# bede/kindel

Hardware: NVIDIA H100
Metric: aligned bases/sec through pileup+consensus (higher is better)
Workload: dtype int32

## Files before the change

include/kindel_b200.h:

```cpp
#ifndef KINDEL_B200_H
#define KINDEL_B200_H

#include <stdint.h>

#ifdef __cplusplus
extern "C" {
#endif

#define KDL_ABI_VERSION 2
#define KDL_NCOL 19
#define KDL_NVOTE_COL 7
#define KDL_COMPLEX 0x80000000u
#define KDL_HARD 0x40000000u
#define KDL_LEN_MASK 0x0000ffffu
#define KDL_NM_SHIFT 16
#define KDL_NM_MASK 0x7fu
#define KDL_TILE 512
#define KDL_FAST_MAXLEN 8192
#define KDL_TILE_MAXOPS 64
#define KDL_TILE_MAXREACH 1024

enum kdl_col {
    KDL_W_A = 0, KDL_W_C, KDL_W_G, KDL_W_T, KDL_W_N,
    KDL_DEL = 5, KDL_INS = 6, KDL_CLIP_STARTS = 7, KDL_CLIP_ENDS = 8,
// ... 39 lines not shown
    const uint32_t* off;
    const uint32_t* qpos;
} kdl_qmask;

typedef struct kdl_diag {
    int32_t status;
    int32_t reserved;
    int64_t read;
    int32_t nibble;
    int32_t op_index;
} kdl_diag;

int kdl_abi_version(void);
const char* kdl_status_string(int status);
int64_t kdl_launch_count(void);

int kdl_pileup(const kdl_batch* batch, int32_t* counts, int64_t n_slots, int32_t* ins_events,
               int32_t* err_flag, void* stream);

#define KDL_PILEUP_FRESH_WEIGHTS 1
#define KDL_PILEUP_ZERO_REST 2
int kdl_pileup_range(const kdl_batch* batch, int32_t* counts, int64_t n_slots, int64_t slot_lo,
                     int64_t slot_hi, int32_t flags, int32_t* ins_events, int32_t* err_flag, void* stream);

int kdl_unmask(const kdl_batch* batch, const kdl_qmask* qmask, int32_t* counts, int64_t n_slots, void* stream);

int kdl_diagnose(const kdl_batch* batch, kdl_diag* diag_dev, void* stream);

int kdl_vote(const int32_t* counts, int64_t n_slots, int64_t min_depth_ceil, uint8_t* calls,
             void* stream);

int kdl_vote_iupac(const int32_t* counts, int64_t n_slots, int64_t min_depth_ceil, double threshold, uint8_t* calls,
                   void* stream);

int kdl_derive(const int32_t* counts, int64_t n_slots, int32_t* out, void* stream);

int kdl_cdr_flags(const int32_t* counts, int64_t n_slots, int64_t slot_lo, int64_t slot_hi,
                  double clip_decay_threshold, uint8_t* flags, uint8_t* bases, void* stream);

int64_t kdl_assemble_scratch_words(int64_t n_slots);
int kdl_assemble(const uint8_t* calls, int64_t n_slots, const int64_t* contig_slot, const int32_t* contig_len,
                 int32_t n_contigs, const int64_t* ins_slot, const uint32_t* ins_off, const uint8_t* ins_bytes,
                 int64_t n_ins, uint32_t* block_sums, uint32_t* offsets, uint8_t* out, void* stream);

int kdl_consensus_qual(const int32_t* counts, const uint8_t* calls, int64_t n_slots, uint8_t* qual, void* stream);

// ... 76 lines not shown
```

kindel_b200/_ffi.py:

```python
from __future__ import annotations

import ctypes as C
import os

from . import build as _build

c_i32p = C.POINTER(C.c_int32)
c_u32p = C.POINTER(C.c_uint32)
c_i64p = C.POINTER(C.c_int64)
c_u8p = C.POINTER(C.c_uint8)

KDL_NCOL = 19
KDL_NVOTE_COL = 7
KDL_COMPLEX = 0x80000000
KDL_HARD = 0x40000000
KDL_LEN_MASK = 0xFFFF
KDL_NM_SHIFT = 16
KDL_NM_MASK = 0x7F
KDL_TILE_MAXOPS = 64
KDL_TILE_MAXREACH = 1024
KDL_TILE = 512
KDL_PILEUP_FRESH_WEIGHTS = 1
KDL_PILEUP_ZERO_REST = 2
KDL_FAST_MAXLEN = 8192
# ... 50 lines not shown
        ("slice_lo", C.c_int64 * 16),
        ("slice_hi", C.c_int64 * 16),
        ("counter", C.c_void_p),
    ]


class KdlDiag(C.Structure):
    _fields_ = [
        ("status", C.c_int32),
        ("reserved", C.c_int32),
        ("read", C.c_int64),
        ("nibble", C.c_int32),
        ("op_index", C.c_int32),
    ]


_PROTOTYPES = {
    "kdl_abi_version": (C.c_int, []),
    "kdl_status_string": (C.c_char_p, [C.c_int]),
    "kdl_launch_count": (C.c_int64, []),
    "kdl_pileup": (C.c_int, [C.POINTER(KdlBatch), C.c_void_p, C.c_int64, C.c_void_p, C.c_void_p, C.c_void_p]),
    "kdl_pileup_range": (C.c_int, [C.POINTER(KdlBatch), C.c_void_p, C.c_int64, C.c_int64, C.c_int64, C.c_int32,
                                   C.c_void_p, C.c_void_p, C.c_void_p]),
    "kdl_diagnose": (C.c_int, [C.POINTER(KdlBatch), C.c_void_p, C.c_void_p]),
    "kdl_unmask": (C.c_int, [C.POINTER(KdlBatch), C.POINTER(KdlQmask), C.c_void_p, C.c_int64, C.c_void_p]),
    "kdl_vote": (C.c_int, [C.c_void_p, C.c_int64, C.c_int64, C.c_void_p, C.c_void_p]),
    "kdl_vote_iupac": (C.c_int, [C.c_void_p, C.c_int64, C.c_int64, C.c_double, C.c_void_p, C.c_void_p]),
    "kdl_derive": (C.c_int, [C.c_void_p, C.c_int64, C.c_void_p, C.c_void_p]),
    "kdl_cdr_flags": (C.c_int, [C.c_void_p, C.c_int64, C.c_int64, C.c_int64, C.c_double, C.c_void_p, C.c_void_p, C.c_void_p]),
    "kdl_assemble_scratch_words": (C.c_int64, [C.c_int64]),
    "kdl_assemble": (C.c_int, [C.c_void_p, C.c_int64, C.c_void_p, C.c_void_p, C.c_int32, C.c_void_p, C.c_void_p,
                               C.c_void_p, C.c_int64, C.c_void_p, C.c_void_p, C.c_void_p, C.c_void_p]),
    "kdl_consensus_qual": (C.c_int, [C.c_void_p, C.c_void_p, C.c_int64, C.c_void_p, C.c_void_p]),
    "kdl_assemble_qual": (C.c_int, [C.c_void_p, C.c_void_p, C.c_int64, C.c_void_p, C.c_void_p, C.c_int64, C.c_void_p,
                                    C.c_void_p]),
    "kdl_variant_scratch_words": (C.c_int64, [C.c_int64]),
    "kdl_variant_count": (C.c_int, [C.c_void_p, C.c_int64, C.c_void_p, C.c_void_p, C.c_int32, C.c_int64, C.c_double,
                                    C.c_void_p, C.c_void_p]),
    "kdl_variant_scatter": (C.c_int, [C.c_void_p, C.c_int64, C.c_void_p, C.c_void_p, C.c_int32, C.c_int64, C.c_double,
                                      C.c_void_p, C.c_int64, C.c_void_p, C.c_void_p, C.c_void_p, C.c_void_p]),
    "kdl_vote_peers": (C.c_int, [C.POINTER(C.c_void_p), C.c_int32, C.c_int64, C.c_int64, C.c_int64, C.c_int64,
                                 C.c_void_p, C.c_void_p, C.c_void_p]),
    "kdl_vote_peers_sparse": (C.c_int, [C.POINTER(C.c_void_p), C.POINTER(C.c_int64), C.POINTER(C.c_int64), C.c_int32,
                                        C.c_int64, C.c_int64, C.c_int64, C.c_int64, C.c_void_p, C.c_void_p, C.c_void_p]),
    "kdl_exchange_signal": (C.c_int, [C.POINTER(KdlExchange), C.c_int32, C.c_void_p]),
    "kdl_exchange_vote": (C.c_int, [C.POINTER(KdlExchange), C.c_int64, C.c_int64, C.c_int32, C.c_void_p]),
# ... 64 lines not shown
```

kindel_b200/csrc/api.cu:

```cuda
#include <atomic>
#include <cstdio>
#include <cstdlib>
#include <cstring>
#include <new>

#include "kdl_common.cuh"
#include "pileup_general.cu"
#include "pileup_simple.cu"
#include "pileup_tile.cu"
#include "pileup_mask.cu"
#include "vote.cu"
#include "assemble.cu"
#include "variants.cu"

namespace {

std::atomic<long long> g_launches{0};

inline int grid_for(long long items, int per_block, int cap) {
    long long g = (items + per_block - 1) / per_block;
    if (g < 1) g = 1;
    if (g > cap) g = cap;
    return (int)g;
}
// ... 11 lines not shown
    const int dev = current_device();
    int n = cache[dev].load(std::memory_order_relaxed);
    if (n <= 0) {
        if (cudaDeviceGetAttribute(&n, cudaDevAttrMultiProcessorCount, dev) != cudaSuccess || n <= 0) n = 132;
        cache[dev].store(n, std::memory_order_relaxed);
    }
    return n;
}

template <int kFlush, bool kCx>
inline int ensure_tile_smem() {
    static std::atomic<int> done[kMaxDevices];
    const int dev = current_device();
    if (done[dev].load(std::memory_order_acquire)) return KDL_OK;
    if (cudaFuncSetAttribute(kdl::pileup_tile_kernel<kFlush, kCx>, cudaFuncAttributeMaxDynamicSharedMemorySize,
                             (int)sizeof(kdl::TileSmem<kdl::TileCfg<kCx>>)) != cudaSuccess)
        return KDL_ERR_CUDA;
    done[dev].store(1, std::memory_order_release);
    return KDL_OK;
}

template <int kFlush, bool kCx>
inline int launch_tile(const kdl_batch& b, int32_t* counts, long long n_slots, long long tile_lo, long long n_tiles,
                       int split, int zero_rest, cudaStream_t st) {
    int rc = ensure_tile_smem<kFlush, kCx>();
    if (rc != KDL_OK) return rc;
    const long long units = n_tiles * split, max_grid = (long long)sm_count() * 2;
    const long long grid = units < max_grid ? units : max_grid;
    kdl::pileup_tile_kernel<kFlush, kCx><<<(unsigned)grid, kdl::W_THREADS, sizeof(kdl::TileSmem<kdl::TileCfg<kCx>>), st>>>(
        b, counts, n_slots, b.tile_index, tile_lo, n_tiles, split, zero_rest);
    return KDL_OK;
}

inline int check_launch() {
    g_launches.fetch_add(1, std::memory_order_relaxed);
    return cudaGetLastError() == cudaSuccess ? KDL_OK : KDL_ERR_CUDA;
}

int validate_batch(const kdl_batch* b) {
    if (!b || b->n_reads < 0 || b->n_contigs < 0 || b->n_hard < 0 || b->n_complex < b->n_hard)
        return KDL_ERR_INVALID_ARG;
    if (b->n_reads > 0 && (!b->ref_start || !b->seq_off || !b->l_seq || !b->seq4 ||
                           !b->contig_read_off || !b->contig_len || !b->contig_slot))
        return KDL_ERR_INVALID_ARG;
    if ((b->n_hard > 0 && !b->hard_idx) || (b->n_complex > 0 && !b->complex_idx)) return KDL_ERR_INVALID_ARG;
    if (b->reach_right < b->max_simple_len || b->reach_left < 0) return KDL_ERR_INVALID_ARG;
    return KDL_OK;
}

}

extern "C" {

int kdl_abi_version(void) { return KDL_ABI_VERSION; }

const char* kdl_status_string(int status) {
    switch (status) {
        case KDL_OK: return "ok";
        case KDL_ERR_INVALID_ARG: return "invalid argument";
        case KDL_ERR_CUDA: return "CUDA error";
        case KDL_ERR_NO_DEVICE: return "no CUDA device";
        case KDL_ERR_INDEX: return "IndexError: read walks off the contig or off its SEQ";
        case KDL_ERR_KEY: return "KeyError: base outside A,C,G,T,N in an M or S op";
        default: return "unknown status";
    }
}

int64_t kdl_launch_count(void) { return g_launches.load(std::memory_order_relaxed); }

int kdl_pileup(const kdl_batch* batch, int32_t* counts, int64_t n_slots, int32_t* ins_events,
               int32_t* err_flag, void* stream) {
    return kdl_pileup_range(batch, counts, n_slots, 0, n_slots, 0, ins_events, err_flag, stream);
}

int kdl_pileup_range(const kdl_batch* batch, int32_t* counts, int64_t n_slots, int64_t slot_lo,
                     int64_t slot_hi, int32_t flags, int32_t* ins_events, int32_t* err_flag, void* stream) {
    int rc = validate_batch(batch);
    if (rc != KDL_OK) return rc;
    if (!counts || !err_flag || n_slots <= 0 || slot_lo < 0 || slot_hi > n_slots || slot_lo > slot_hi)
        return KDL_ERR_INVALID_ARG;
    const bool tileable = (n_slots % KDL_TILE) == 0 && (slot_lo % KDL_TILE) == 0 && (slot_hi % KDL_TILE) == 0;
    if ((slot_lo & 3) || (slot_hi & 3)) return KDL_ERR_INVALID_ARG;
    cudaStream_t st = (cudaStream_t)stream;
    const int cap = sm_count() * 8;
    const bool has_tile_reads = batch->n_reads > batch->n_hard;
    const bool tiled = has_tile_reads && tileable && batch->reads_sorted && batch->tile_index &&
                       batch->reach_right > 0 && batch->reach_right <= KDL_FAST_MAXLEN + KDL_TILE_MAXREACH;
    const bool fresh = (flags & KDL_PILEUP_FRESH_WEIGHTS) != 0;
    const long long tile_lo = slot_lo / KDL_TILE, n_tiles = (slot_hi - slot_lo) / KDL_TILE;
    int split = 1;
    if (tiled && n_tiles > 0) {
        const long long slots = (long long)sm_count() * 2;
        if (n_tiles < slots) {
            long long want = (slots + n_tiles - 1) / n_tiles;
            const long long deep = batch->n_reads / (n_tiles * 256);
            if (want > deep) want = deep;
            split = (int)(want < 1 ? 1 : (want > 32 ? 32 : want));
        }
        if (const char* ev = getenv("KDL_SPLIT")) { const int v = atoi(ev); if (v >= 1 && v <= 64) split = v; }
    }
    bool cx_by_atomics = (batch->n_complex - batch->n_hard) * 16 < batch->n_reads;
    if (const char* ev = getenv("KDL_CX")) cx_by_atomics = !strcmp(ev, "atomics") ? true : (!strcmp(ev, "pieces") ? false : cx_by_atomics);
    const int zero_in_k1 = (tiled && split == 1 && fresh && n_tiles > 0 && (flags & KDL_PILEUP_ZERO_REST)) ? 1 : 0;
    const int zero_from = (fresh && !(tiled && split == 1)) ? 0 : 5;
    const int zero_to = ((flags & KDL_PILEUP_ZERO_REST) && !zero_in_k1) ? KDL_NCOL : 5;
    if (zero_to > zero_from && slot_hi > slot_lo) {
        kdl::zero_cols_kernel<<<sm_count() * 4, 256, 0, st>>>(counts, n_slots, zero_from, zero_to, slot_lo, slot_hi);
        if ((rc = check_launch()) != KDL_OK) return rc;
    }
    if (batch->n_reads == 0) return KDL_OK;
    if (tiled) {
        if (n_tiles > 0) {
            kdl::tile_index_kernel<<<(unsigned)((n_tiles * 32 + 255) / 256), 256, 0, st>>>(*batch, tile_lo, n_tiles,
                                                                                          batch->tile_index);
            if ((rc = check_launch()) != KDL_OK) return rc;
            const bool cx = batch->n_complex > batch->n_hard && !cx_by_atomics;
            if (split > 1) {
                rc = cx ? launch_tile<kdl::F_ATOMIC, true>(*batch, counts, n_slots, tile_lo, n_tiles, split, 0, st)
                        : launch_tile<kdl::F_ATOMIC, false>(*batch, counts, n_slots, tile_lo, n_tiles, split, 0, st);
            } else if (fresh) {
                rc = cx ? launch_tile<kdl::F_STORE, true>(*batch, counts, n_slots, tile_lo, n_tiles, 1, zero_in_k1, st)
                        : launch_tile<kdl::F_STORE, false>(*batch, counts, n_slots, tile_lo, n_tiles, 1, zero_in_k1, st);
            } else {
                rc = cx ? launch_tile<kdl::F_ADD, true>(*batch, counts, n_slots, tile_lo, n_tiles, 1, 0, st)
                        : launch_tile<kdl::F_ADD, false>(*batch, counts, n_slots, tile_lo, n_tiles, 1, 0, st);
            }
            if (rc != KDL_OK) return rc;
            if ((rc = check_launch()) != KDL_OK) return rc;
        }
        if (batch->n_complex > batch->n_hard) {
            if (cx_by_atomics)
                kdl::pileup_events_kernel<8><<<(unsigned)((batch->n_complex + 31) / 32), 256, 0, st>>>(
                    *batch, counts, n_slots, ins_events, 1);
            else
                kdl::pileup_events_kernel<1><<<(unsigned)((batch->n_complex + 255) / 256), 256, 0, st>>>(
                    *batch, counts, n_slots, ins_events, 0);
            if ((rc = check_launch()) != KDL_OK) return rc;
        }
        if (batch->n_hard > 0) {
            const int grid = grid_for(batch->n_hard, 8, cap);
            kdl::pileup_general_kernel<<<grid, 256, 0, st>>>(*batch, batch->hard_idx, batch->n_hard, counts, n_slots,
                                                            ins_events, err_flag);
            if ((rc = check_launch()) != KDL_OK) return rc;
        }
    } else {
        if (batch->n_reads > batch->n_complex) {
            const int grid = grid_for(batch->n_reads, 8, cap);
            kdl::pileup_simple_atomic_kernel<<<grid, 256, 0, st>>>(*batch, counts, n_slots, err_flag);
            if ((rc = check_launch()) != KDL_OK) return rc;
        }
        if (batch->n_complex > 0) {
            const int grid = grid_for(batch->n_reads, 8, cap);
            kdl::pileup_general_kernel<<<grid, 256, 0, st>>>(*batch, nullptr, batch->n_reads, counts, n_slots,
                                                            ins_events, err_flag);
            if ((rc = check_launch()) != KDL_OK) return rc;
        }
    }
    return KDL_OK;
}

int kdl_unmask(const kdl_batch* batch, const kdl_qmask* qmask, int32_t* counts, int64_t n_slots, void* stream) {
    int rc = validate_batch(batch);
    if (rc != KDL_OK) return rc;
    if (!qmask || !counts || n_slots <= 0 || qmask->n_reads < 0 || qmask->n_bases < 0 || qmask->n_reads > batch->n_reads)
        return KDL_ERR_INVALID_ARG;
    if (qmask->n_reads == 0) return KDL_OK;
    if (!qmask->read_idx || !qmask->off || !qmask->qpos) return KDL_ERR_INVALID_ARG;
    const long long grid = (qmask->n_reads + kdl::kQThreads - 1) / kdl::kQThreads;
    kdl::unmask_kernel<<<(unsigned)grid, kdl::kQThreads, 0, (cudaStream_t)stream>>>(*batch, *qmask, counts, n_slots);
    return check_launch();
}

int kdl_diagnose(const kdl_batch* batch, kdl_diag* diag_dev, void* stream) {
    int rc = validate_batch(batch);
    if (rc != KDL_OK) return rc;
    if (!diag_dev) return KDL_ERR_INVALID_ARG;
    cudaStream_t st = (cudaStream_t)stream;
// ... 268 lines not shown
```

kindel_b200/csrc/kdl_common.cuh:

```cuda
#pragma once
#include <cuda_runtime.h>
#include <stdint.h>

#include "../../include/kindel_b200.h"

#ifndef KDL_HOST_EMU
#define KDL_DYNAMIC_SMEM(name) extern __shared__ __align__(16) unsigned char name[]
#else
#define KDL_DYNAMIC_SMEM(name) extern unsigned char name[]
#endif

namespace kdl {

__device__ __forceinline__ int nib2col(int nib) {
    const unsigned long long lut = 0x4FFFFFF3FFF2F10FULL;
    int v = (int)((lut >> (nib * 4)) & 0xF);
    return v == 0xF ? -1 : v;
}

__device__ __forceinline__ int nibble_at(const uint32_t* __restrict__ seq, long long q) {
    return (int)((seq[q >> 3] >> (28 - 4 * (int)(q & 7))) & 0xFu);
}

__device__ __forceinline__ long long complex_len(uint32_t lraw) {
    return (lraw & KDL_HARD) ? (long long)(lraw & 0x3fffffffu) : (long long)(lraw & KDL_LEN_MASK);
}

__device__ __forceinline__ long long pyindex(long long i, long long n) {
    if (i < 0) i += n;
    return (i < 0 || i >= n) ? -1 : i;
}

__device__ __forceinline__ int find_contig(const int64_t* __restrict__ off, int n_contigs, long long r) {
    int lo = 0, hi = n_contigs;
    while (lo < hi) {
        int mid = (lo + hi) >> 1;
        if (off[mid + 1] > r) hi = mid; else lo = mid + 1;
    }
    return lo;
}

__device__ __forceinline__ int base_vote(int a, int c, int g, int t, int n, int* freq, int* raw_base) {
    int best = a, code = 0;
    if (t > best) { best = t; code = 3; }
    if (g > best) { best = g; code = 2; }
    if (c > best) { best = c; code = 1; }
    if (n > best) { best = n; code = 4; }
    const int ties = (a == best) + (c == best) + (g == best) + (t == best) + (n == best);
    if (best == 0) code = 4;
    *freq = best;
    *raw_base = code;
    return (best != 0 && ties > 1) ? 4 : code;
}

__device__ __forceinline__ unsigned vote_slot(int a, int c, int g, int t, int n, int del, int ins,
                                              long long depth_next, long long min_depth_ceil) {
    const long long depth = (long long)a + c + g + t;
    if (2ll * del > depth) return (1u << 4) | 4u;
    if (depth < min_depth_ceil) return (2u << 4) | 4u;
    const long long thr = depth < depth_next ? depth : depth_next;
    const unsigned change = (2ll * ins > thr) ? 3u : 0u;
    int freq, raw;
// ... 53 lines not shown
```

kindel_b200/csrc/pileup_general.cu:

```cuda
#include "kdl_common.cuh"

namespace kdl {

__global__ void __launch_bounds__(256)
pileup_general_kernel(kdl_batch b, const uint32_t* __restrict__ list, long long n_list, int32_t* __restrict__ counts,
                      long long n_slots, int32_t* __restrict__ ins_events, int32_t* __restrict__ err_flag) {
    const int lane = threadIdx.x & 31;
    const long long warp0 = ((long long)blockIdx.x * blockDim.x + threadIdx.x) >> 5;
    const long long n_warps = ((long long)gridDim.x * blockDim.x) >> 5;
    bool bad = false;

    for (long long j = warp0; j < n_list; j += n_warps) {
        const long long r = list ? (long long)list[j] : j;
        const uint32_t lraw = (uint32_t)b.l_seq[r];
        if (!(lraw & KDL_COMPLEX)) continue;
        const int c = find_contig(b.contig_read_off, b.n_contigs, r);
        const long long L = b.contig_len[c];
        const long long base = b.contig_slot[c];
        const long long lseq = complex_len(lraw);
        const uint32_t* __restrict__ seq = b.seq4 + (size_t)b.seq_off[r];
        const uint32_t* __restrict__ blk = seq + ((lseq + 7) >> 3);
        const uint32_t c0 = 0, c1 = blk[0];
        const uint32_t* __restrict__ cig = blk + 2;
        long long r_pos = b.ref_start[r];
        long long q_pos = 0;
        uint32_t evt = blk[1];

        for (uint32_t i = c0; i < c1; ++i) {
            const uint32_t cg = cig[i];
            const long long len = cg >> 4;
            const int op = cg & 0xF;
            if (op == 0 || op == 7 || op == 8) {
                for (long long k = lane; k < len; k += 32) {
                    const long long q = q_pos + k;
                    const long long idx = pyindex(r_pos + k, L);
                    if (q >= lseq || idx < 0) { bad = true; continue; }
                    const int col = nib2col(nibble_at(seq, q));
                    if (col < 0) { bad = true; continue; }
                    atomicAdd(counts + (long long)(KDL_W_A + col) * n_slots + base + idx, 1);
                }
                r_pos += len;
                q_pos += len;
            } else if (op == 1) {
                if (lane == 0) {
                    const long long idx = pyindex(r_pos, L + 1);
                    if (idx < 0) {
                        bad = true;
                    } else {
                        atomicAdd(counts + (long long)KDL_INS * n_slots + base + idx, 1);
                        if (ins_events) {
                            int4 e = make_int4((int)(base + idx), (int)r, (int)q_pos, (int)len);
                            reinterpret_cast<int4*>(ins_events)[evt] = e;
                        }
                    }
                }
                evt += 1;
                q_pos += len;
            } else if (op == 2) {
                for (long long k = lane; k < len; k += 32) {
                    const long long idx = pyindex(r_pos + k, L + 1);
                    if (idx < 0) { bad = true; continue; }
                    atomicAdd(counts + (long long)KDL_DEL * n_slots + base + idx, 1);
                }
                r_pos += len;
            } else if (op == 4) {
                if (i == c0) {
                    if (lane == 0) {
                        const long long idx = pyindex(r_pos, L + 1);
                        if (idx < 0) bad = true;
                        else atomicAdd(counts + (long long)KDL_CLIP_ENDS * n_slots + base + idx, 1);
                    }
                    for (long long g = lane; g < len; g += 32) {
                        if (g >= lseq) { bad = true; continue; }
                        const long long rel = r_pos - len + g;
                        if (rel < 0) continue;
                        if (rel >= L) { bad = true; continue; }
                        const int col = nib2col(nibble_at(seq, g));
                        if (col < 0) { bad = true; continue; }
                        atomicAdd(counts + (long long)(KDL_CEW_A + col) * n_slots + base + rel, 1);
                    }
                    q_pos += len;
                } else {
                    if (lane == 0) {
                        const long long idx = pyindex(r_pos - 1, L + 1);
                        if (idx < 0) bad = true;
                        else atomicAdd(counts + (long long)KDL_CLIP_STARTS * n_slots + base + idx, 1);
                    }
                    long long n_adv = L - r_pos;
                    n_adv = n_adv < 0 ? 0 : (n_adv > len ? len : n_adv);
                    for (long long k = lane; k < n_adv; k += 32) {
                        const long long q = q_pos + k;
                        const long long idx = pyindex(r_pos + k, L);
                        if (q >= lseq || idx < 0) { bad = true; continue; }
                        const int col = nib2col(nibble_at(seq, q));
                        if (col < 0) { bad = true; continue; }
                        atomicAdd(counts + (long long)(KDL_CSW_A + col) * n_slots + base + idx, 1);
                    }
                    if (n_adv < len && q_pos + n_adv >= lseq) bad = true;
                    r_pos += n_adv;
                    q_pos += n_adv;
                }
            }
        }
    }
    if (bad) atomicOr(err_flag, 1);
}

template <int kLanes>
__global__ void __launch_bounds__(256)
pileup_events_kernel(kdl_batch b, int32_t* __restrict__ counts, long long n_slots, int32_t* __restrict__ ins_events,
                     int with_m) {
    const int lane = (int)(threadIdx.x % kLanes);
    constexpr int kStep = kLanes;
    const long long gtid = (long long)blockIdx.x * blockDim.x + threadIdx.x;
    const long long j = gtid / kLanes;
    if (j >= b.n_complex) return;
    const long long r = (long long)b.complex_idx[j];
    const uint32_t lraw = (uint32_t)b.l_seq[r];
    if ((lraw & (KDL_COMPLEX | KDL_HARD)) != KDL_COMPLEX) return;
    const int c = find_contig(b.contig_read_off, b.n_contigs, r);
    const long long slot0 = b.contig_slot[c];
    int32_t* __restrict__ tab = counts + slot0;
    const uint32_t* __restrict__ seq = b.seq4 + (size_t)b.seq_off[r];
    const uint32_t* __restrict__ blk = seq + (((lraw & KDL_LEN_MASK) + 7) >> 3);
    const int n_ops = (int)blk[0];
    uint32_t evt = blk[1];
    const uint32_t* __restrict__ ops = blk + 2;
    long long r_pos = b.ref_start[r];
    int q_pos = 0;
    for (int o = 0; o < n_ops; ++o) {
        const uint32_t cg = ops[o];
        const int len = (int)(cg >> 4);
        const int op = (int)(cg & 0xF);
        if (op == 0 || op == 7 || op == 8) {
            if (with_m)
                for (int d = lane; d < len; d += kStep)
                    atomicAdd(tab + (long long)(KDL_W_A + nib2col(nibble_at(seq, q_pos + d))) * n_slots + r_pos + d, 1);
            r_pos += len;
            q_pos += len;
        } else if (op == 1) {
            if (lane == 0) {
                atomicAdd(tab + (long long)KDL_INS * n_slots + r_pos, 1);
                if (ins_events)
                    reinterpret_cast<int4*>(ins_events)[evt] = make_int4((int)(slot0 + r_pos), (int)r, q_pos, len);
            }
            evt += 1;
            q_pos += len;
        } else if (op == 2) {
            for (int d = lane; d < len; d += kStep) atomicAdd(tab + (long long)KDL_DEL * n_slots + r_pos + d, 1);
            r_pos += len;
        } else if (op == 4) {
            if (o == 0) {
                if (lane == 0) atomicAdd(tab + (long long)KDL_CLIP_ENDS * n_slots + r_pos, 1);
                for (int g = lane; g < len; g += kStep) {
                    const long long rel = r_pos - len + g;
                    if (rel >= 0) atomicAdd(tab + (long long)(KDL_CEW_A + nib2col(nibble_at(seq, g))) * n_slots + rel, 1);
                }
                q_pos += len;
            } else {
                if (lane == 0) atomicAdd(tab + (long long)KDL_CLIP_STARTS * n_slots + r_pos - 1, 1);
                for (int d = lane; d < len; d += kStep)
                    atomicAdd(tab + (long long)(KDL_CSW_A + nib2col(nibble_at(seq, q_pos + d))) * n_slots + r_pos + d, 1);
                r_pos += len;
                q_pos += len;
            }
        }
    }
}

__device__ unsigned long long diagnose_read(const kdl_batch& b, long long j) {
    const long long r = (long long)b.hard_idx[j];
    const int c = find_contig(b.contig_read_off, b.n_contigs, r);
    const long long L = b.contig_len[c];
    const long long lseq = complex_len((uint32_t)b.l_seq[r]);
    const uint32_t* __restrict__ seq = b.seq4 + (size_t)b.seq_off[r];
    const uint32_t* __restrict__ blk = seq + ((lseq + 7) >> 3);
    const uint32_t c0 = 0, c1 = blk[0];
    const uint32_t* __restrict__ cig = blk + 2;
    long long r_pos = b.ref_start[r], q_pos = 0;
#define KDL_FAIL(kind, nib)                                                                     \
    return ((unsigned long long)r << 24) | ((unsigned long long)(kind) << 20) |                 \
           ((unsigned long long)(nib) << 16) | (unsigned long long)((i - c0) > 0xFFFF ? 0xFFFF : (i - c0))
// ... 73 lines not shown
```

kindel_b200/csrc/pileup_tile.cu:

```cuda
#include "tile_common.cuh"

namespace kdl {

constexpr int W_CONSUMERS = 8;
constexpr int W_PRODUCERS = 4;
#ifndef KDL_W_STAGES
#define KDL_W_STAGES 2
#endif
constexpr int W_STAGES = KDL_W_STAGES;
constexpr int W_THREADS = 32 * (W_CONSUMERS + W_PRODUCERS);
constexpr int W_PT = 32 * W_PRODUCERS;
template <bool kCx> struct TileRegs { static constexpr int kProducer = kCx ? 64 : 56, kConsumer = 88; };
static_assert(W_PT * TileRegs<true>::kProducer + 32 * W_CONSUMERS * TileRegs<true>::kConsumer <= W_THREADS * 80 &&
              W_PT * TileRegs<false>::kProducer + 32 * W_CONSUMERS * TileRegs<false>::kConsumer <= W_THREADS * 80,
              "register pool of the CTA");

template <bool kCx> struct TileCfg;
#if KDL_W_STAGES == 2
template <> struct TileCfg<false> {
    static constexpr int kRmax = 512;
    static constexpr int kCapW = 9728;
    static constexpr int kPcap = 0;
};
template <> struct TileCfg<true> {
// ... 47 lines not shown
template <class C>
struct TileSmem {
    TileStage<C> st[W_STAGES];
    int raw[3][C::kRmax];
    unsigned short queue[W_CONSUMERS][C::kPcap ? 64 : 4];
    int scan[W_PRODUCERS * 4 + 4];
    uint64_t full[W_STAGES];
    uint64_t landed[W_STAGES];
    uint64_t empty[W_STAGES];
};
static_assert(sizeof(TileSmem<TileCfg<false>>) <= 113 * 1024 && sizeof(TileSmem<TileCfg<true>>) <= 113 * 1024,
              "K1 must fit two CTAs per SM (228 KB of shared memory per SM, 1 KB of it reserved per CTA)");
static_assert(offsetof(TileStage<TileCfg<false>>, diff) % 16 == 0 && sizeof(TileStage<TileCfg<false>>) % 16 == 0 &&
              offsetof(TileStage<TileCfg<true>>, diff) % 16 == 0 && sizeof(TileStage<TileCfg<true>>) % 16 == 0 &&
              offsetof(TileStage<TileCfg<true>>, px) % 16 == 0 && offsetof(TileStage<TileCfg<true>>, meta) % 16 == 0,
              "128-bit shared accesses of the metadata and the pieces, 64-bit ones of the difference array");
static_assert(TileCfg<false>::kRmax % W_PT == 0 && TileCfg<true>::kRmax % W_PT == 0, "reads per producer thread");
static_assert(TileCfg<true>::kPcap >= KDL_TILE_MAXOPS && TileCfg<true>::kPcap < 1024, "one read's pieces fit; 10-bit piece slot");

template <int kFlush, bool kCx>
__global__ void __launch_bounds__(W_THREADS, 2)
pileup_tile_kernel(kdl_batch b, int32_t* __restrict__ counts, long long n_slots,
                   const uint32_t* __restrict__ tile_index, long long tile_lo, long long n_tiles, int split,
                   int zero_rest) {
    KDL_DYNAMIC_SMEM(smem_raw);
    using C = TileCfg<kCx>;
    using Smem = TileSmem<C>;
    using Stage = TileStage<C>;
    constexpr int W_RMAX = C::kRmax, W_CAPW = C::kCapW, W_PCAP = C::kPcap;
    constexpr bool kFresh = kFlush == F_STORE;
    constexpr int kAdd = kFlush == F_ATOMIC ? F_ATOMIC : F_ADD;
    Smem& sm = *reinterpret_cast<Smem*>(smem_raw);
    const int tid = threadIdx.x, lane = tid & 31, warp = tid >> 5;
    const int maxlen = b.max_simple_len;
    const long long n_units = n_tiles * split;

    if (tid == 0) {
        for (int s = 0; s < W_STAGES; ++s) {
            mbar_init(&sm.full[s], W_PRODUCERS);
            mbar_init(&sm.landed[s], 1);
            mbar_init(&sm.empty[s], W_CONSUMERS);
        }
    }
    for (int s = 0; s < W_STAGES; ++s) {
        for (int k = tid; k < KDL_TILE + 32; k += W_THREADS) sm.st[s].diff[k] = 0;
        if (tid < W_CONSUMERS) sm.st[s].carry[tid] = 0;
        if (tid == 0) sm.st[s].px[W_PCAP] = make_int4(0x10000000, (int)smem_u32(sm.st[s].seq), 0, 0);
// ... 478 lines not shown
        if (flags & ITEM_LAST) {
            if (blocks_since_flush & 1) acc.template ripple<3>(pend8);
            int covacc[8];
            {
                const int both = dacc.x + dacc.y;
                int run = both;
#pragma unroll
                for (int d = 1; d < 32; d <<= 1) {
                    const int o = __shfl_up_sync(0xffffffffu, run, d);
                    if (lane >= d) run += o;
                }
                const int c0 = cacc + run - dacc.y, c1 = cacc + run;
#pragma unroll
                for (int k = 0; k < 4; ++k) {
                    const int src = 4 * (lane & 7) + k;
                    covacc[2 * k] = __shfl_sync(0xffffffffu, c0, src);
                    covacc[2 * k + 1] = __shfl_sync(0xffffffffu, c1, src);
                }
                dacc = make_int2(0, 0);
                cacc = 0;
            }
            if (kFresh && !stored) flush_window<F_STORE, true>(acc, rawacc, covacc, counts, n_slots, tile_slot + wlo, lane);
            else flush_window<kAdd, true>(acc, rawacc, covacc, counts, n_slots, tile_slot + wlo, lane);
            if (kFresh && zero_rest) {
                int32_t* z = counts + tile_slot + wlo + 8 * (lane & 7);
                for (int col = 5 + quarter; col < KDL_NCOL; col += 4) {
                    int4* zp = reinterpret_cast<int4*>(z + (long long)col * n_slots);
                    zp[0] = make_int4(0, 0, 0, 0);
                    zp[1] = make_int4(0, 0, 0, 0);
                }
            }
            blocks_since_flush = 0;
        }
    }
}

}
```

kindel_b200/csrc/tile_common.cuh:

```cuda
#pragma once
#include <stddef.h>

#include "kdl_common.cuh"

namespace kdl {

constexpr int F_WIN = 64;
constexpr int F_P = 8;
constexpr int F_FLUSH_BLOCKS = 31;
static_assert(F_FLUSH_BLOCKS % 2 == 1, "the counting loop folds exactly one pending carry at a mid-window flush");

constexpr int F_IDX = 8;

struct Search {
    long long a, e, p;
    bool live;
};

__device__ __forceinline__ Search search_begin(const kdl_batch& b, long long g) {
    Search s;
    s.live = false;
    s.a = s.e = 0;
    s.p = 0;
    if (b.n_contigs == 0) return s;
// ... 314 lines not shown
#pragma unroll
            for (int k = 0; k < 8; ++k)
                if (nn[k]) atomicAdd(ncol + k, nn[k]);
        }
        return;
    }
    v0.x += cv[0] - nn[0]; v0.y += cv[1] - nn[1]; v0.z += cv[2] - nn[2]; v0.w += cv[3] - nn[3];
    v1.x += cv[4] - nn[4]; v1.y += cv[5] - nn[5]; v1.z += cv[6] - nn[6]; v1.w += cv[7] - nn[7];
    dst[0] = v0;
    dst[1] = v1;
    if (q == 0 && (kFinal || kMode == F_STORE)) {
        int4* dn = reinterpret_cast<int4*>(counts + (long long)KDL_W_N * n_slots + s);
        int4 n0 = make_int4(0, 0, 0, 0), n1 = n0;
        if (kMode == F_ADD) { n0 = dn[0]; n1 = dn[1]; }
        n0.x += nn[0]; n0.y += nn[1]; n0.z += nn[2]; n0.w += nn[3];
        n1.x += nn[4]; n1.y += nn[5]; n1.z += nn[6]; n1.w += nn[7];
        dn[0] = n0;
        dn[1] = n1;
    }
}

__global__ void __launch_bounds__(256)
zero_cols_kernel(int32_t* __restrict__ counts, long long n_slots, int col_lo, int col_hi, long long slot_lo,
                 long long slot_hi) {
    const long long per_col = (slot_hi - slot_lo) >> 2;
    const long long total = per_col * (col_hi - col_lo);
    for (long long v = (long long)blockIdx.x * blockDim.x + threadIdx.x; v < total;
         v += (long long)gridDim.x * blockDim.x) {
        const long long col = col_lo + v / per_col, off = v % per_col;
        reinterpret_cast<int4*>(counts + col * n_slots + slot_lo)[off] = make_int4(0, 0, 0, 0);
    }
}

}
```

kindel_b200/engine.py:

```python
from __future__ import annotations

import ctypes as C
import math
from dataclasses import dataclass

import numpy as np
import torch

from . import _ffi
from .bamio import NIBBLES, ReadBatch


def require_cuda(device=None) -> torch.device:
    if not torch.cuda.is_available():
        raise RuntimeError(
            "kindel_b200 needs a CUDA device (H100, sm_90a): the pileup and the vote exist only as "
            "CUDA kernels and there is no CPU fallback")
    if device is None:
        device = torch.device("cuda", torch.cuda.current_device())
    return torch.device(device)


def _stream_ptr(device) -> int:
    return int(torch.cuda.current_stream(device).cuda_stream)
# ... 82 lines not shown
    ptr = {f: int(t.data_ptr()) for f, t in tensors.items()}
    if host.n_masked:
        qmask = make_qmask(host, ptr)
    return DeviceBatch(host=host, device=device, tensors=tensors, struct=make_struct(host, ptr), qmask=qmask)


def raise_like_reference(status: int, read: int, nibble: int, op_index: int):
    if status == _ffi.KDL_ERR_KEY:
        exc = KeyError(NIBBLES[nibble])
    else:
        exc = IndexError("list index out of range (read %d, CIGAR op %d walks off its contig or its SEQ)"
                         % (read, op_index))
    exc.kdl_read = int(read)
    raise exc


class CountTable:

    def __init__(self, n_slots: int, device, tensor: torch.Tensor = None):
        self.n_slots = n_slots
        self.device = device
        self.t = tensor if tensor is not None else torch.zeros((_ffi.KDL_NCOL, n_slots), dtype=torch.int32,
                                                                device=device)
        self.dirty = None
        self.dirty_rest = False


def _tile_align(lo: int, hi: int, n_slots: int):
    t = _ffi.KDL_TILE
    return max(0, lo // t * t), min(n_slots, (hi + t - 1) // t * t)


def pileup(dbatch: DeviceBatch, counts: torch.Tensor = None, check: bool = True, table: CountTable = None,
           slot_range=None):
    lib = _ffi.load()
    dev = dbatch.device
    n_slots = dbatch.n_slots
    with torch.cuda.device(dev):
        events = dbatch.tensors.get("_events")
        if events is None:
            events = dbatch.tensors["_events"] = torch.empty((max(dbatch.host.n_events, 1), 4), dtype=torch.int32,
                                                             device=dev)
            dbatch.tensors["_flag"] = torch.zeros(4, dtype=torch.int32, device=dev)
        flag = dbatch.tensors["_flag"]
        if check:
            flag.zero_()
        if table is not None:
            counts = table.t
            lo, hi = slot_range if slot_range is not None else (0, n_slots)
            if table.dirty is not None:
                lo, hi = min(lo, table.dirty[0]), max(hi, table.dirty[1])
            lo, hi = _tile_align(lo, hi, n_slots)
            flags = _ffi.KDL_PILEUP_FRESH_WEIGHTS | (_ffi.KDL_PILEUP_ZERO_REST if table.dirty_rest else 0)
            rc = lib.kdl_pileup_range(C.byref(dbatch.struct), counts.data_ptr(), n_slots, lo, hi, flags,
                                      events.data_ptr(), flag.data_ptr(), _stream_ptr(dev))
            table.dirty = (lo, hi)
            table.dirty_rest = dbatch.host.n_complex > 0
        else:
            if counts is None:
                counts = torch.zeros((_ffi.KDL_NCOL, n_slots), dtype=torch.int32, device=dev)
            rc = lib.kdl_pileup(C.byref(dbatch.struct), counts.data_ptr(), n_slots, events.data_ptr(),
                                flag.data_ptr(), _stream_ptr(dev))
        _ffi.check(rc, "kdl_pileup")
        if dbatch.qmask is not None:
            assert table is None or table.dirty_rest or dbatch.host.n_complex == 0
            rc = lib.kdl_unmask(C.byref(dbatch.struct), C.byref(dbatch.qmask), counts.data_ptr(), n_slots,
                                _stream_ptr(dev))
            _ffi.check(rc, "kdl_unmask")
        if check and int(flag[0].item()) != 0:
            diagnose_and_raise(dbatch)
    return counts, events[: dbatch.host.n_events]


def diagnose_and_raise(dbatch: DeviceBatch):
    lib = _ffi.load()
    dev = dbatch.device
    diag = torch.zeros(6, dtype=torch.int32, device=dev)
    rc = lib.kdl_diagnose(C.byref(dbatch.struct), diag.data_ptr(), _stream_ptr(dev))
    _ffi.check(rc, "kdl_diagnose")
    raw = diag.cpu().numpy().tobytes()
# ... 200 lines not shown
```

Before: 1567 billion.

## Track dirty sparse columns with a bitmap to skip redundant zeroing

Adds a per-64-slot dirty bitmap for the sparse count columns (deletions, insertions, clips and clip-weight columns). The complex-read kernels mark it with atomicOr as they write, and the tile kernel and zero kernel use it so that only previously written 8-slot groups get cleared on table reuse. The aim is to cut the write bandwidth spent zeroing 14 mostly-empty columns on every reused pileup. In exchange, the complex-read kernels pay extra atomics, there is more bookkeeping, and a saturation fallback covers batches with many complex reads.

Measured after the change: 1784 billion (median of 6 runs). +13.9%, better.

```diff
diff --git a/include/kindel_b200.h b/include/kindel_b200.h
--- a/include/kindel_b200.h
+++ b/include/kindel_b200.h
@@ -85,6 +85,9 @@
 #define KDL_PILEUP_ZERO_REST 2
 int kdl_pileup_range(const kdl_batch* batch, int32_t* counts, int64_t n_slots, int64_t slot_lo,
                      int64_t slot_hi, int32_t flags, int32_t* ins_events, int32_t* err_flag, void* stream);
+
+int kdl_pileup_range_map(const kdl_batch* batch, int32_t* counts, int64_t n_slots, int64_t slot_lo, int64_t slot_hi,
+                         int32_t flags, uint32_t* dirty_map, int32_t* ins_events, int32_t* err_flag, void* stream);
 
 int kdl_unmask(const kdl_batch* batch, const kdl_qmask* qmask, int32_t* counts, int64_t n_slots, void* stream);
 
diff --git a/kindel_b200/_ffi.py b/kindel_b200/_ffi.py
--- a/kindel_b200/_ffi.py
+++ b/kindel_b200/_ffi.py
@@ -96,6 +96,8 @@
     "kdl_pileup": (C.c_int, [C.POINTER(KdlBatch), C.c_void_p, C.c_int64, C.c_void_p, C.c_void_p, C.c_void_p]),
     "kdl_pileup_range": (C.c_int, [C.POINTER(KdlBatch), C.c_void_p, C.c_int64, C.c_int64, C.c_int64, C.c_int32,
                                    C.c_void_p, C.c_void_p, C.c_void_p]),
+    "kdl_pileup_range_map": (C.c_int, [C.POINTER(KdlBatch), C.c_void_p, C.c_int64, C.c_int64, C.c_int64, C.c_int32,
+                                       C.c_void_p, C.c_void_p, C.c_void_p, C.c_void_p]),
     "kdl_diagnose": (C.c_int, [C.POINTER(KdlBatch), C.c_void_p, C.c_void_p]),
     "kdl_unmask": (C.c_int, [C.POINTER(KdlBatch), C.POINTER(KdlQmask), C.c_void_p, C.c_int64, C.c_void_p]),
     "kdl_vote": (C.c_int, [C.c_void_p, C.c_int64, C.c_int64, C.c_void_p, C.c_void_p]),
diff --git a/kindel_b200/csrc/api.cu b/kindel_b200/csrc/api.cu
--- a/kindel_b200/csrc/api.cu
+++ b/kindel_b200/csrc/api.cu
@@ -57,13 +57,13 @@
 
 template <int kFlush, bool kCx>
 inline int launch_tile(const kdl_batch& b, int32_t* counts, long long n_slots, long long tile_lo, long long n_tiles,
-                       int split, int zero_rest, cudaStream_t st) {
+                       int split, int zero_rest, uint32_t* dirty_map, uint32_t map_after, cudaStream_t st) {
     int rc = ensure_tile_smem<kFlush, kCx>();
     if (rc != KDL_OK) return rc;
     const long long units = n_tiles * split, max_grid = (long long)sm_count() * 2;
     const long long grid = units < max_grid ? units : max_grid;
     kdl::pileup_tile_kernel<kFlush, kCx><<<(unsigned)grid, kdl::W_THREADS, sizeof(kdl::TileSmem<kdl::TileCfg<kCx>>), st>>>(
-        b, counts, n_slots, b.tile_index, tile_lo, n_tiles, split, zero_rest);
+        b, counts, n_slots, b.tile_index, tile_lo, n_tiles, split, zero_rest, dirty_map, map_after);
     return KDL_OK;
 }
 
@@ -110,9 +110,15 @@
 
 int kdl_pileup_range(const kdl_batch* batch, int32_t* counts, int64_t n_slots, int64_t slot_lo,
                      int64_t slot_hi, int32_t flags, int32_t* ins_events, int32_t* err_flag, void* stream) {
+    return kdl_pileup_range_map(batch, counts, n_slots, slot_lo, slot_hi, flags, nullptr, ins_events, err_flag, stream);
+}
+
+int kdl_pileup_range_map(const kdl_batch* batch, int32_t* counts, int64_t n_slots, int64_t slot_lo, int64_t slot_hi,
+                         int32_t flags, uint32_t* dirty_map, int32_t* ins_events, int32_t* err_flag, void* stream) {
     int rc = validate_batch(batch);
     if (rc != KDL_OK) return rc;
-    if (!counts || !err_flag || n_slots <= 0 || slot_lo < 0 || slot_hi > n_slots || slot_lo > slot_hi)
+    if (!counts || !err_flag || n_slots <= 0 || slot_lo < 0 || slot_hi > n_slots || slot_lo > slot_hi ||
+        (reinterpret_cast<uintptr_t>(dirty_map) & 15))
         return KDL_ERR_INVALID_ARG;
     const bool tileable = (n_slots % KDL_TILE) == 0 && (slot_lo % KDL_TILE) == 0 && (slot_hi % KDL_TILE) == 0;
     if ((slot_lo & 3) || (slot_hi & 3)) return KDL_ERR_INVALID_ARG;
@@ -139,10 +145,18 @@
     const int zero_in_k1 = (tiled && split == 1 && fresh && n_tiles > 0 && (flags & KDL_PILEUP_ZERO_REST)) ? 1 : 0;
     const int zero_from = (fresh && !(tiled && split == 1)) ? 0 : 5;
     const int zero_to = ((flags & KDL_PILEUP_ZERO_REST) && !zero_in_k1) ? KDL_NCOL : 5;
-    if (zero_to > zero_from && slot_hi > slot_lo) {
-        kdl::zero_cols_kernel<<<sm_count() * 4, 256, 0, st>>>(counts, n_slots, zero_from, zero_to, slot_lo, slot_hi);
+    const bool zero_pass = zero_to > zero_from && slot_hi > slot_lo;
+    const bool k1_stores = tiled && split == 1 && fresh && n_tiles > 0;
+    const bool saturate = dirty_map && batch->n_complex > 0 && batch->n_complex * 16 >= batch->n_reads &&
+                          (k1_stores || zero_pass);
+    uint32_t* mark_map = saturate ? nullptr : dirty_map;
+    if (zero_pass) {
+        uint32_t* zmap = saturate || (zero_from <= 5 && zero_to == KDL_NCOL) ? dirty_map : nullptr;
+        kdl::zero_cols_kernel<<<sm_count() * 4, 256, 0, st>>>(counts, n_slots, zero_from, zero_to, slot_lo, slot_hi,
+                                                              zmap, saturate ? ~0u : 0u);
         if ((rc = check_launch()) != KDL_OK) return rc;
     }
+    const uint32_t map_after = saturate && k1_stores ? ~0u : 0u;
     if (batch->n_reads == 0) return KDL_OK;
     if (tiled) {
         if (n_tiles > 0) {
@@ -151,14 +165,16 @@
             if ((rc = check_launch()) != KDL_OK) return rc;
             const bool cx = batch->n_complex > batch->n_hard && !cx_by_atomics;
             if (split > 1) {
-                rc = cx ? launch_tile<kdl::F_ATOMIC, true>(*batch, counts, n_slots, tile_lo, n_tiles, split, 0, st)
-                        : launch_tile<kdl::F_ATOMIC, false>(*batch, counts, n_slots, tile_lo, n_tiles, split, 0, st);
+                rc = cx ? launch_tile<kdl::F_ATOMIC, true>(*batch, counts, n_slots, tile_lo, n_tiles, split, 0, nullptr, 0, st)
+                        : launch_tile<kdl::F_ATOMIC, false>(*batch, counts, n_slots, tile_lo, n_tiles, split, 0, nullptr, 0, st);
             } else if (fresh) {
-                rc = cx ? launch_tile<kdl::F_STORE, true>(*batch, counts, n_slots, tile_lo, n_tiles, 1, zero_in_k1, st)
-                        : launch_tile<kdl::F_STORE, false>(*batch, counts, n_slots, tile_lo, n_tiles, 1, zero_in_k1, st);
+                rc = cx ? launch_tile<kdl::F_STORE, true>(*batch, counts, n_slots, tile_lo, n_tiles, 1, zero_in_k1, dirty_map,
+                                                          map_after, st)
+                        : launch_tile<kdl::F_STORE, false>(*batch, counts, n_slots, tile_lo, n_tiles, 1, zero_in_k1, dirty_map,
+                                                           map_after, st);
             } else {
-                rc = cx ? launch_tile<kdl::F_ADD, true>(*batch, counts, n_slots, tile_lo, n_tiles, 1, 0, st)
-                        : launch_tile<kdl::F_ADD, false>(*batch, counts, n_slots, tile_lo, n_tiles, 1, 0, st);
+                rc = cx ? launch_tile<kdl::F_ADD, true>(*batch, counts, n_slots, tile_lo, n_tiles, 1, 0, nullptr, 0, st)
+                        : launch_tile<kdl::F_ADD, false>(*batch, counts, n_slots, tile_lo, n_tiles, 1, 0, nullptr, 0, st);
             }
             if (rc != KDL_OK) return rc;
             if ((rc = check_launch()) != KDL_OK) return rc;
@@ -166,16 +182,16 @@
         if (batch->n_complex > batch->n_hard) {
             if (cx_by_atomics)
                 kdl::pileup_events_kernel<8><<<(unsigned)((batch->n_complex + 31) / 32), 256, 0, st>>>(
-                    *batch, counts, n_slots, ins_events, 1);
+                    *batch, counts, n_slots, ins_events, 1, mark_map);
             else
                 kdl::pileup_events_kernel<1><<<(unsigned)((batch->n_complex + 255) / 256), 256, 0, st>>>(
-                    *batch, counts, n_slots, ins_events, 0);
+                    *batch, counts, n_slots, ins_events, 0, mark_map);
             if ((rc = check_launch()) != KDL_OK) return rc;
         }
         if (batch->n_hard > 0) {
             const int grid = grid_for(batch->n_hard, 8, cap);
             kdl::pileup_general_kernel<<<grid, 256, 0, st>>>(*batch, batch->hard_idx, batch->n_hard, counts, n_slots,
-                                                            ins_events, err_flag);
+                                                            ins_events, err_flag, mark_map);
             if ((rc = check_launch()) != KDL_OK) return rc;
         }
     } else {
@@ -187,7 +203,7 @@
         if (batch->n_complex > 0) {
             const int grid = grid_for(batch->n_reads, 8, cap);
             kdl::pileup_general_kernel<<<grid, 256, 0, st>>>(*batch, nullptr, batch->n_reads, counts, n_slots,
-                                                            ins_events, err_flag);
+                                                            ins_events, err_flag, mark_map);
             if ((rc = check_launch()) != KDL_OK) return rc;
         }
     }
diff --git a/kindel_b200/csrc/kdl_common.cuh b/kindel_b200/csrc/kdl_common.cuh
--- a/kindel_b200/csrc/kdl_common.cuh
+++ b/kindel_b200/csrc/kdl_common.cuh
@@ -38,6 +38,33 @@
         if (off[mid + 1] > r) hi = mid; else lo = mid + 1;
     }
     return lo;
+}
+
+__device__ __forceinline__ void mark_dirty(uint32_t* __restrict__ map, int col, int n_col, long long s0, long long s1) {
+    if (s0 >= s1) return;
+    const uint32_t bytes = ((1u << n_col) - 1u) << (col - KDL_DEL);
+    uint32_t* rec = map + 4 * (s0 >> 6);
+    int lo = (int)(s0 & 63), left = (int)(s1 - s0);
+    do {
+        const int hi = left < 64 - lo ? lo + left : 64;
+        const uint32_t sec = ((2u << ((hi - 1) >> 3)) - 1u) & ~((1u << (lo >> 3)) - 1u);
+#pragma unroll
+        for (int k = 0; k < 4; ++k) {
+            const uint32_t nib = (bytes >> (4 * k)) & 0xFu;
+            const uint32_t v = sec * ((nib & 1u) | ((nib & 2u) << 7) | ((nib & 4u) << 14) | ((nib & 8u) << 21));
+            if (v) atomicOr(rec + k, v);
+        }
+        left -= hi - lo;
+        lo = 0;
+        rec += 4;
+    } while (left > 0);
+}
+
+__device__ __forceinline__ void mark_dirty_py(uint32_t* __restrict__ map, int col, int n_col, long long base,
+                                              long long lo, long long hi, long long n) {
+    const long long a = lo > -n ? lo : -n, e = hi < 0 ? hi : 0;
+    if (a < e) mark_dirty(map, col, n_col, base + a + n, base + e + n);
+    mark_dirty(map, col, n_col, base + (lo > 0 ? lo : 0), base + (hi < n ? hi : n));
 }
 
 __device__ __forceinline__ int base_vote(int a, int c, int g, int t, int n, int* freq, int* raw_base) {
diff --git a/kindel_b200/csrc/pileup_general.cu b/kindel_b200/csrc/pileup_general.cu
--- a/kindel_b200/csrc/pileup_general.cu
+++ b/kindel_b200/csrc/pileup_general.cu
@@ -4,8 +4,10 @@
 
 __global__ void __launch_bounds__(256)
 pileup_general_kernel(kdl_batch b, const uint32_t* __restrict__ list, long long n_list, int32_t* __restrict__ counts,
-                      long long n_slots, int32_t* __restrict__ ins_events, int32_t* __restrict__ err_flag) {
+                      long long n_slots, int32_t* __restrict__ ins_events, int32_t* __restrict__ err_flag,
+                      uint32_t* __restrict__ dirty_map = nullptr) {
     const int lane = threadIdx.x & 31;
+    const bool marks = dirty_map != nullptr && lane == 0;
     const long long warp0 = ((long long)blockIdx.x * blockDim.x + threadIdx.x) >> 5;
     const long long n_warps = ((long long)gridDim.x * blockDim.x) >> 5;
     bool bad = false;
@@ -42,6 +44,7 @@
                 r_pos += len;
                 q_pos += len;
             } else if (op == 1) {
+                if (marks) mark_dirty_py(dirty_map, KDL_INS, 1, base, r_pos, r_pos + 1, L + 1);
                 if (lane == 0) {
                     const long long idx = pyindex(r_pos, L + 1);
                     if (idx < 0) {
@@ -57,6 +60,7 @@
                 evt += 1;
                 q_pos += len;
             } else if (op == 2) {
+                if (marks) mark_dirty_py(dirty_map, KDL_DEL, 1, base, r_pos, r_pos + len, L + 1);
                 for (long long k = lane; k < len; k += 32) {
                     const long long idx = pyindex(r_pos + k, L + 1);
                     if (idx < 0) { bad = true; continue; }
@@ -65,6 +69,11 @@
                 r_pos += len;
             } else if (op == 4) {
                 if (i == c0) {
+                    if (marks) {
+                        mark_dirty_py(dirty_map, KDL_CLIP_ENDS, 1, base, r_pos, r_pos + 1, L + 1);
+                        mark_dirty(dirty_map, KDL_CEW_A, 5, base + (r_pos - len > 0 ? r_pos - len : 0),
+                                   base + (r_pos < L ? r_pos : L));
+                    }
                     if (lane == 0) {
                         const long long idx = pyindex(r_pos, L + 1);
                         if (idx < 0) bad = true;
@@ -88,6 +97,10 @@
                     }
                     long long n_adv = L - r_pos;
                     n_adv = n_adv < 0 ? 0 : (n_adv > len ? len : n_adv);
+                    if (marks) {
+                        mark_dirty_py(dirty_map, KDL_CLIP_STARTS, 1, base, r_pos - 1, r_pos, L + 1);
+                        mark_dirty_py(dirty_map, KDL_CSW_A, 5, base, r_pos, r_pos + n_adv, L);
+                    }
                     for (long long k = lane; k < n_adv; k += 32) {
                         const long long q = q_pos + k;
                         const long long idx = pyindex(r_pos + k, L);
@@ -109,7 +122,7 @@
 template <int kLanes>
 __global__ void __launch_bounds__(256)
 pileup_events_kernel(kdl_batch b, int32_t* __restrict__ counts, long long n_slots, int32_t* __restrict__ ins_events,
-                     int with_m) {
+                     int with_m, uint32_t* __restrict__ dirty_map = nullptr) {
     const int lane = (int)(threadIdx.x % kLanes);
     constexpr int kStep = kLanes;
     const long long gtid = (long long)blockIdx.x * blockDim.x + threadIdx.x;
@@ -128,6 +141,7 @@
     const uint32_t* __restrict__ ops = blk + 2;
     long long r_pos = b.ref_start[r];
     int q_pos = 0;
+    const bool marks = dirty_map != nullptr && lane == 0;
     for (int o = 0; o < n_ops; ++o) {
         const uint32_t cg = ops[o];
         const int len = (int)(cg >> 4);
@@ -140,6 +154,7 @@
             q_pos += len;
         } else if (op == 1) {
             if (lane == 0) {
+                if (marks) mark_dirty(dirty_map, KDL_INS, 1, slot0 + r_pos, slot0 + r_pos + 1);
                 atomicAdd(tab + (long long)KDL_INS * n_slots + r_pos, 1);
                 if (ins_events)
                     reinterpret_cast<int4*>(ins_events)[evt] = make_int4((int)(slot0 + r_pos), (int)r, q_pos, len);
@@ -147,10 +162,15 @@
             evt += 1;
             q_pos += len;
         } else if (op == 2) {
+            if (marks) mark_dirty(dirty_map, KDL_DEL, 1, slot0 + r_pos, slot0 + r_pos + len);
             for (int d = lane; d < len; d += kStep) atomicAdd(tab + (long long)KDL_DEL * n_slots + r_pos + d, 1);
             r_pos += len;
         } else if (op == 4) {
             if (o == 0) {
+                if (marks) {
+                    mark_dirty(dirty_map, KDL_CLIP_ENDS, 1, slot0 + r_pos, slot0 + r_pos + 1);
+                    mark_dirty(dirty_map, KDL_CEW_A, 5, slot0 + (r_pos - len > 0 ? r_pos - len : 0), slot0 + r_pos);
+                }
                 if (lane == 0) atomicAdd(tab + (long long)KDL_CLIP_ENDS * n_slots + r_pos, 1);
                 for (int g = lane; g < len; g += kStep) {
                     const long long rel = r_pos - len + g;
@@ -158,6 +178,10 @@
                 }
                 q_pos += len;
             } else {
+                if (marks) {
+                    mark_dirty(dirty_map, KDL_CLIP_STARTS, 1, slot0 + r_pos - 1, slot0 + r_pos);
+                    mark_dirty(dirty_map, KDL_CSW_A, 5, slot0 + r_pos, slot0 + r_pos + len);
+                }
                 if (lane == 0) atomicAdd(tab + (long long)KDL_CLIP_STARTS * n_slots + r_pos - 1, 1);
                 for (int d = lane; d < len; d += kStep)
                     atomicAdd(tab + (long long)(KDL_CSW_A + nib2col(nibble_at(seq, q_pos + d))) * n_slots + r_pos + d, 1);
diff --git a/kindel_b200/csrc/pileup_tile.cu b/kindel_b200/csrc/pileup_tile.cu
--- a/kindel_b200/csrc/pileup_tile.cu
+++ b/kindel_b200/csrc/pileup_tile.cu
@@ -93,7 +93,7 @@
 __global__ void __launch_bounds__(W_THREADS, 2)
 pileup_tile_kernel(kdl_batch b, int32_t* __restrict__ counts, long long n_slots,
                    const uint32_t* __restrict__ tile_index, long long tile_lo, long long n_tiles, int split,
-                   int zero_rest) {
+                   int zero_rest, uint32_t* __restrict__ dirty_map = nullptr, uint32_t map_after = 0u) {
     KDL_DYNAMIC_SMEM(smem_raw);
     using C = TileCfg<kCx>;
     using Smem = TileSmem<C>;
@@ -618,13 +618,28 @@
             }
             if (kFresh && !stored) flush_window<F_STORE, true>(acc, rawacc, covacc, counts, n_slots, tile_slot + wlo, lane);
             else flush_window<kAdd, true>(acc, rawacc, covacc, counts, n_slots, tile_slot + wlo, lane);
+            uint4* mrec = kFresh && dirty_map ? reinterpret_cast<uint4*>(dirty_map) + ((tile_slot + wlo) >> 6) : nullptr;
+            uint4 rec = make_uint4(~0u, ~0u, ~0u, ~0u);
             if (kFresh && zero_rest) {
                 int32_t* z = counts + tile_slot + wlo + 8 * (lane & 7);
-                for (int col = 5 + quarter; col < KDL_NCOL; col += 4) {
-                    int4* zp = reinterpret_cast<int4*>(z + (long long)col * n_slots);
-                    zp[0] = make_int4(0, 0, 0, 0);
-                    zp[1] = make_int4(0, 0, 0, 0);
-                }
+                if (mrec) rec = *mrec;
+                const int sh = 8 * quarter + (lane & 7);
+                const uint32_t mine = ((rec.x >> sh) & 1u) | (((rec.y >> sh) & 1u) << 1) | (((rec.z >> sh) & 1u) << 2) |
+                                      (((rec.w >> sh) & 1u) << 3);
+#pragma unroll
+                for (int k = 0; k < 4; ++k) {
+                    const int col = 5 + quarter + 4 * k;
+                    if (col < KDL_NCOL && ((mine >> k) & 1u)) {
+                        int4* zp = reinterpret_cast<int4*>(z + (long long)col * n_slots);
+                        zp[0] = make_int4(0, 0, 0, 0);
+                        zp[1] = make_int4(0, 0, 0, 0);
+                    }
+                }
+                __syncwarp();
+            }
+            if (mrec && lane == 0) {
+                const bool differs = rec.x != map_after || rec.y != map_after || rec.z != map_after || rec.w != map_after;
+                if (zero_rest ? differs : map_after != 0u) *mrec = make_uint4(map_after, map_after, map_after, map_after);
             }
             blocks_since_flush = 0;
         }
diff --git a/kindel_b200/csrc/tile_common.cuh b/kindel_b200/csrc/tile_common.cuh
--- a/kindel_b200/csrc/tile_common.cuh
+++ b/kindel_b200/csrc/tile_common.cuh
@@ -360,14 +360,21 @@
 
 __global__ void __launch_bounds__(256)
 zero_cols_kernel(int32_t* __restrict__ counts, long long n_slots, int col_lo, int col_hi, long long slot_lo,
-                 long long slot_hi) {
+                 long long slot_hi, uint32_t* __restrict__ dirty_map = nullptr, uint32_t map_fill = 0u) {
     const long long per_col = (slot_hi - slot_lo) >> 2;
     const long long total = per_col * (col_hi - col_lo);
-    for (long long v = (long long)blockIdx.x * blockDim.x + threadIdx.x; v < total;
-         v += (long long)gridDim.x * blockDim.x) {
+    const long long gtid = (long long)blockIdx.x * blockDim.x + threadIdx.x, stride = (long long)gridDim.x * blockDim.x;
+    for (long long v = gtid; v < total; v += stride) {
         const long long col = col_lo + v / per_col, off = v % per_col;
         reinterpret_cast<int4*>(counts + col * n_slots + slot_lo)[off] = make_int4(0, 0, 0, 0);
     }
-}
-
-}
+    if (dirty_map) {
+        const bool whole = map_fill == 0 && slot_hi != n_slots;
+        const long long w_lo = map_fill ? slot_lo >> 6 : (slot_lo + 63) >> 6;
+        const long long w_hi = whole ? slot_hi >> 6 : (slot_hi + 63) >> 6;
+        for (long long w = w_lo + gtid; w < w_hi; w += stride)
+            reinterpret_cast<uint4*>(dirty_map)[w] = make_uint4(map_fill, map_fill, map_fill, map_fill);
+    }
+}
+
+}
diff --git a/kindel_b200/engine.py b/kindel_b200/engine.py
--- a/kindel_b200/engine.py
+++ b/kindel_b200/engine.py
@@ -128,8 +128,20 @@
         self.device = device
         self.t = tensor if tensor is not None else torch.zeros((_ffi.KDL_NCOL, n_slots), dtype=torch.int32,
                                                                 device=device)
+        self.dirty_map = torch.full((4 * ((n_slots + 63) // 64),), 0 if tensor is None else -1, dtype=torch.int32,
+                                    device=device)
         self.dirty = None
-        self.dirty_rest = False
+        self._dirty_rest = False
+
+    @property
+    def dirty_rest(self) -> bool:
+        return self._dirty_rest
+
+    @dirty_rest.setter
+    def dirty_rest(self, value: bool):
+        if value:
+            self.dirty_map.fill_(-1)
+        self._dirty_rest = bool(value)
 
 
 def _tile_align(lo: int, hi: int, n_slots: int):
@@ -158,10 +170,11 @@
                 lo, hi = min(lo, table.dirty[0]), max(hi, table.dirty[1])
             lo, hi = _tile_align(lo, hi, n_slots)
             flags = _ffi.KDL_PILEUP_FRESH_WEIGHTS | (_ffi.KDL_PILEUP_ZERO_REST if table.dirty_rest else 0)
-            rc = lib.kdl_pileup_range(C.byref(dbatch.struct), counts.data_ptr(), n_slots, lo, hi, flags,
-                                      events.data_ptr(), flag.data_ptr(), _stream_ptr(dev))
+            rc = lib.kdl_pileup_range_map(C.byref(dbatch.struct), counts.data_ptr(), n_slots, lo, hi, flags,
+                                          table.dirty_map.data_ptr(), events.data_ptr(), flag.data_ptr(),
+                                          _stream_ptr(dev))
             table.dirty = (lo, hi)
-            table.dirty_rest = dbatch.host.n_complex > 0
+            table._dirty_rest = dbatch.host.n_complex > 0
         else:
             if counts is None:
                 counts = torch.zeros((_ffi.KDL_NCOL, n_slots), dtype=torch.int32, device=dev)
```
